# tranthai189765/MARL-Snake

Measured on AMD Instinct MI355X. Metric: env-steps/sec whole-node, 65536×(20×20, 4 snakes), random actions; 1→8 GPU, higher is better.
Workload: dtype u8

## Files before the change

marl-snake_amd/csrc/snake_capi.cpp:

```cpp
#include <stdarg.h>
#include <stdio.h>
#include <stdlib.h>
#include <string.h>

#include <math.h>

#include <algorithm>
#include <map>
#include <mutex>
#include <tuple>
#include <vector>

#include "snake_internal.h"

#ifndef SNAKE_SPAWN_PRIO_SMALL
#define SNAKE_SPAWN_PRIO_SMALL 3
#endif

namespace snake {

static thread_local char g_err[512];

void set_error(const char *fmt, ...)
{
    va_list ap;
    va_start(ap, fmt);
    vsnprintf(g_err, sizeof g_err, fmt, ap);
    va_end(ap);
}

static int64_t round_up(int64_t x, int64_t m) { return (x + m - 1) / m * m; }

static int pow2_at_least(int x)
{
    int p = 1;
    while (p < x) p <<= 1;
    return p;
}

static int check_cfg(const snake_cfg *c)
{
    if (!c) { set_error("cfg is NULL"); return SNAKE_E_CONFIG; }
    if (c->height < 3 || c->height > 255 || c->width < 3 || c->width > 255) {
        set_error("height/width must be in [3, 255] (got %d x %d)", c->height, c->width);
        return SNAKE_E_CONFIG;
    }
    if (c->num_snakes < 1 || c->num_snakes > kMaxSnakes) {
        set_error("num_snakes must be in [1, %d] (got %d)", kMaxSnakes, c->num_snakes);
        return SNAKE_E_CONFIG;
    }
    if (c->snake_length < 2 || c->snake_length > 63) {
        set_error("snake_length must be in [2, 63] (got %d)", c->snake_length);
        return SNAKE_E_CONFIG;
    }
    if (c->snake_length * c->num_snakes > kWave) {
        set_error("num_snakes * snake_length must be <= 64 (got %d)", c->snake_length * c->num_snakes);
        return SNAKE_E_CONFIG;
    }
    if (c->vision_range < 0 || 2 * c->vision_range + 1 > 255) {
        set_error("vision_range must be None/0 or in [1, 127] (got %d)", c->vision_range);
        return SNAKE_E_CONFIG;
    }
    if (c->frame_stack < 1 || c->frame_stack > 16) {
        set_error("frame_stack must be in [1, 16] (got %d)", c->frame_stack);
        return SNAKE_E_CONFIG;
    }
    if (c->observer != 0 && c->observer != 1) {
        set_error("observer must be 'snake' or 'human'");
        return SNAKE_E_CONFIG;
    }
    if (c->num_fruits < 1 || c->num_fruits > kMaxFruits) {
        set_error("num_fruits must be in [1, %d] (got %d)", kMaxFruits, c->num_fruits);
        return SNAKE_E_CONFIG;
    }
    int interior = (c->height - 2) * (c->width - 2);
    if (interior < c->num_snakes * c->snake_length + 1) {
        set_error("grid too small for %d snakes of length %d", c->num_snakes, c->snake_length);
        return SNAKE_E_CONFIG;
    }
    return SNAKE_OK;
}

struct Dfs {
    int H, W, L;
    std::vector<uint8_t> empty;
    std::vector<int16_t> *out;
    int64_t count = 0;
    int path[64];
    int dir_state[64];
};

static bool in_path(const Dfs &d, int n, int cell)
{
    for (int i = 0; i < n; i++)
        if (d.path[i] == cell) return true;
    return false;
}

static bool head_blocked(const Dfs &d, int n, int extra)
// ... 231 lines not shown
    }
    o->obs = N * S * oh * ow * 8 * fs;
    o->rew = N * S * 8;
    o->done = N * S;
    o->ep_done = N;
    o->rank = N * S * 4;
    o->ep_stats = N * 4 * S * 8;
    o->err = N * 4;
    if (o->n_cand > 65535) {
        set_error("%lld spawn poses: more than the 65535 the reset scratch indexes",
                  (long long)o->n_cand);
        return SNAKE_E_CONFIG;
    }
    if (o->n_cand < S) {
        set_error("only %lld spawn poses for %lld snakes", (long long)o->n_cand, (long long)S);
        return SNAKE_E_CONFIG;
    }
    int64_t samples = 0;
    const double pd = disjoint_prob(c->height, c->width, c->snake_length, (int)S, &samples);
    if (pd < kMinDisjoint) {
        set_error("%dx%d board too crowded: %lld snakes of length %d are disjoint in only "
                  "%.2g of the spawn draws (Monte-Carlo estimate: %lld of %lld sampled draws; the limit is %.0e; "
                  "the reference would retry ~%.0f permutations per reset)",
                  c->height, c->width, (long long)S, c->snake_length, pd, (long long)llround(pd * samples),
                  (long long)samples, kMinDisjoint, pd > 0 ? 1.0 / pd : 1e30);
        return SNAKE_E_CONFIG;
    }
    return SNAKE_OK;
}

int build_kcfg(const snake_cfg *c, int64_t N, int64_t n_cand, KCfg *k)
{
    snake_layout lay;
    int rc = layout_of(c, N, &lay);
    if (rc) return rc;
    if (n_cand != lay.n_cand) {
        set_error("spawn-pose table has %lld rows, expected %lld", (long long)n_cand,
                  (long long)lay.n_cand);
        return SNAKE_E_ARG;
    }
    memset(k, 0, sizeof *k);
    k->N = (int)N;
    k->H = c->height; k->W = c->width; k->HW = c->height * c->width;
    k->S = c->num_snakes; k->L = c->snake_length; k->vr = c->vision_range;
    k->fs = c->frame_stack; k->observer = c->observer; k->num_fruits = c->num_fruits;
    k->coop = c->coop ? 1 : 0; k->autoreset = c->autoreset == 2 ? 2 : (c->autoreset ? 1 : 0);
    k->oh = lay.obs_h; k->ow = lay.obs_w;
    k->units = k->S * k->oh * k->ow * k->fs;
    k->grid_stride = lay.grid_stride; k->ring_cap = lay.ring_cap; k->n_cand = (int)lay.n_cand;
    k->cs = (k->HW + kWave - 1) / kWave;
    k->ring_bytes = k->fs * k->grid_stride;
    int64_t a = 128;
    k->adv_f = (int)(a % k->fs); a /= k->fs;
    k->adv_j = (int)(a % k->ow); a /= k->ow;
    k->adv_i = (int)(a % k->oh); a /= k->oh;
    k->adv_k = (int)a;
    int off = 0;
    k->lds_frames = off; off += (int)round_up((int64_t)k->fs * k->grid_stride, 16);
    k->lds_centers = off; off += (int)round_up(4 * k->fs * kMaxSnakes, 16);
    k->lds_fruit = off; off += (int)round_up(2 * kMaxFruits, 16);
    {
        const int64_t P = (int64_t)k->oh * k->ow * 8 * k->fs;
        int g = 0;
        if ((int64_t)k->S * P <= kStageMax) {
            g = k->S;
        } else {
            g = (int)std::min<int64_t>(k->S, kStageMax / P);
            if (P % 16 != 0) g &= ~1;
        }
        k->enc_group = g;
        k->lds_stage = off;
        k->lds_worker = off;
        if (g > 0) off += (int)round_up(g * P, 16);
        const uint64_t fsoh = (uint64_t)k->fs * k->oh, oh = (uint64_t)k->oh;
        k->mag_fsoh = (uint32_t)(((1ull << 32) + fsoh - 1) / fsoh);
        k->mag_oh = (uint32_t)(((1ull << 32) + oh - 1) / oh);
        k->mag_W = (uint32_t)(((1ull << 32) + k->W - 1) / k->W);
        const uint64_t n16 = (uint64_t)k->grid_stride / 16;
        k->mag_n16 = (uint32_t)(((1ull << 32) + n16 - 1) / n16);
    }
    k->link_stride = (int)round_up(k->n_cand, 4) + kWave;
    int jbytes = (int)round_up(2 * ((int64_t)k->n_cand + kWave), 16);
    k->link_in_lds = jbytes <= kJarrLdsMax;
    if (k->link_in_lds && N <= 32768 && !bg_of(c, n_cand, N) && 4 * (int64_t)k->link_stride <= kJarrLdsMax) {
        k->link32 = 1;
        jbytes = 4 * k->link_stride;
    }
    k->reset_slots = (int)std::min<int64_t>(N, kResetSlots);
    const bool bg = bg_of(c, n_cand, N);
    const bool bg_small = bg && n_cand <= 8192 && N <= 8192;
    if (bg_small) k->reset_slots = (int)std::min<int64_t>(N, 512);
    k->spawn_prio = N <= 32768 && !bg ? SNAKE_SPAWN_PRIO_SMALL : 1;
    k->encode_prio = bg ? 0 : 2;
    {
        const int ms_min = k->S <= 4 ? 4 : (k->S <= 8 ? 8 : 16);
        k->logic_ms = N <= 8192 ? std::max(ms_min, 8) : ms_min;
    }
    auto logic_lds = [&](int G) {
        const int E = kWave / G;
        return (int)round_up((int64_t)E * k->grid_stride + 2 * kMaxFruits + E * G * 4 * 4 + E * G * 2, 16);
    };
    while (k->logic_ms < 16 && logic_lds(k->logic_ms) > kLdsLimit) k->logic_ms *= 2;
    k->lds_logic = logic_lds(k->logic_ms);
    if (k->lds_logic > kLdsLimit) {
        set_error("%dx%d board: k_logic's %d frames per wave (%d bytes) do not fit the %d-byte LDS", k->H, k->W,
                  kWave / k->logic_ms, k->lds_logic, kLdsLimit);
        return SNAKE_E_CONFIG;
    }
    k->logic_wpb = 4 * (int64_t)k->lds_logic <= kLdsLimit ? 4 : 1;
    k->q_envs_per_block = kWave / k->logic_ms;
    k->q_cap = (int)queue_cap(N, k->q_envs_per_block);
    k->spawn_thr = spawn_thr_of(c);
    if (bg_small && c->spawn_ahead == 0 && !c->coop && k->spawn_thr == 3) k->spawn_thr = 4;
    k->bg = bg ? 1 : 0;
    k->spawn_slots = (int)std::min<int64_t>(N, bg_small ? 512 : kResetSlots);
#ifndef SNAKE_BG_TRIES_SMALL
#define SNAKE_BG_TRIES_SMALL 2
#endif
    k->bg_tries = bg_small ? SNAKE_BG_TRIES_SMALL : 1;
    k->spawn_tries = 1;
    k->lds_obs_bytes = off;
    {
        const LeanGeom g = lean_geom(c);
        k->lean = g.lean; k->lp = g.lp; k->pw = g.pw; k->pframe = g.pframe;
        k->lds_lean_bytes = g.lds_lean_bytes; k->ups = g.ups; k->rowl = g.rowl;
        k->mag_ups = g.mag_ups; k->mag_rowl = g.mag_rowl; k->mag_fs = g.mag_fs; k->mag_wpr = g.mag_wpr;
        const int64_t fdw = (int64_t)k->fs * k->HW / 4;
        int t = 0;
        k->tbl_base = (int)round_up((int64_t)k->fs * k->pframe, 16); t = k->tbl_base + 8 * k->fs * kMaxSnakes;
        k->tbl_pat = t; t += 8 * k->S * 160;
        k->tbl_desc = t; t += (int)round_up(4 * (int64_t)k->units, 16);
        k->lds_tbl_bytes = t;
        k->tbl = g.exact && !g.lean && fdw <= 8 * kWave && t <= 40 * 1024 ? 1 : 0;
        if (g.lean && t <= 48 * 1024) k->tbl = 1;
    }
    k->enc_per_wave = k->lean ? 2 : (N >= 16384 && k->ring_bytes <= 8 * 1024 ? 2 : 1);
    if (k->tbl) k->enc_per_wave = k->lean ? 2 : 4;
    k->lds_link = k->lds_stage;
    k->lds_bytes = k->link_in_lds ? std::max(off, k->lds_stage + jbytes) : off;
    if (k->lds_bytes > 64 * 1024) {
        set_error("grid ring of %d bytes per env does not fit the LDS budget", k->ring_bytes);
        return SNAKE_E_CONFIG;
    }
    {
        const int E = kWave / k->logic_ms;
        k->nlg = (int)((N + E - 1) / E);
        k->fused = c->autoreset == 1 && k->tbl && !k->lean && !k->bg && k->fs == 1 && k->S <= 4 &&
                   k->enc_per_wave == 4 && E % 4 == 0 && (k->link32 || k->link_in_lds) ? 1 : 0;
        const int64_t fb = fused_base(N), groups = round_up((N + 3) / 4, 4);
        k->fu_ldone = fb;
        k->fu_done = fb + kQShards * kQSpread;
        k->fu_claim = k->fu_done + groups;
        k->fu_hoff = k->fu_claim + groups;
        k->epoch = 0;
    }
    k->rf = c->rew_fruit; k->rk = c->rew_kill; k->rl = c->rew_lose; k->rw = c->rew_win;
    k->rt = c->rew_time; k->max_steps = c->max_episode_steps;
    return SNAKE_OK;
}

static int check_state(const KCfg &k, const snake_state *st, bool need_all)
{
    if (!st || !st->grid || !st->snake || !st->body || !st->env || !st->ctr || !st->stats ||
        !st->mt || !st->cand) {
        set_error("snake_state has a NULL buffer");
        return SNAKE_E_ARG;
    }
    if (!st->resetq || !st->spawn) {
        set_error("snake_state.resetq / spawn is NULL");
        return SNAKE_E_ARG;
    }
    if ((!k.link_in_lds || (k.lean && k.autoreset == 1)) && !st->jscratch) {
        set_error("snake_state.jscratch is required for this config (n_cand=%d)", k.n_cand);
        return SNAKE_E_ARG;
    }
    (void)need_all;
    return SNAKE_OK;
}

static int check_out(const snake_out *o, bool step)
{
    if (!o || !o->obs) { set_error("snake_out.obs is NULL"); return SNAKE_E_ARG; }
    if (step && (!o->rew || !o->done || !o->ep_done || !o->rank || !o->ep_stats || !o->err)) {
        set_error("snake_out has a NULL step buffer");
        return SNAKE_E_ARG;
    }
    return SNAKE_OK;
}

static int64_t n_cand_of(const snake_cfg *c)
{
    snake_layout lay;
    if (layout_of(c, 1, &lay)) return -1;
    return lay.n_cand;
}

static int plan_cached(const snake_cfg *c, int64_t N, KCfg *k)
{
    struct Entry {
        snake_cfg cfg;
        int64_t n;
        KCfg k;
    };
    thread_local Entry memo[8];
    thread_local int used = 0, next = 0;
    if (!c) { set_error("cfg is NULL"); return SNAKE_E_CONFIG; }
    for (int i = 0; i < used; i++) {
        if (memo[i].n == N && memcmp(&memo[i].cfg, c, sizeof *c) == 0) {
            *k = memo[i].k;
            return SNAKE_OK;
        }
    }
    int rc = build_kcfg(c, N, n_cand_of(c), k);
    if (rc) return rc;
    Entry &e = memo[next];
    e.cfg = *c;
    e.n = N;
    e.k = *k;
    next = (next + 1) % 8;
    used = used < 8 ? used + 1 : 8;
    return SNAKE_OK;
}
// ... 103 lines not shown
```

marl-snake_amd/csrc/snake_internal.h:

```cpp
#pragma once
#include <stdint.h>

#include "../../include/snake_env.h"

namespace snake {

constexpr int kWave = 64;
constexpr int kMtN = 624;
constexpr int kMaxSnakes = 16;
constexpr int kMaxFruits = 64;
constexpr int kEnvRec = 8;
constexpr int kJarrLdsMax = 36864;
constexpr int kLdsLimit = 160 * 1024;
constexpr int kResetSlots = 2048;
constexpr int kQShards = 64;
constexpr int kStageMax = 8192;
constexpr int kSpawnStride = 672;
constexpr int kSpawnPos = 624;
constexpr int kSpawnCells = 625;
constexpr int kQSpread = 32;
constexpr int kClaimShards = 16;
constexpr int kNumQ = 3;
constexpr int kQClaim = kNumQ * kQShards;
constexpr int kQDone = kQClaim + kClaimShards;
constexpr int kQSpClaim = kQDone + 1;
constexpr int kQSpDone = kQSpClaim + kClaimShards;
constexpr int kQSpGen = kQSpDone + 1;
constexpr int kQCount = kQSpGen + 1;
constexpr int kQCounters = kQCount * kQSpread;
#ifndef SNAKE_QSETS
#define SNAKE_QSETS 4
#endif
constexpr int kQSets = SNAKE_QSETS;
static_assert(kQSets == 2 || kQSets == 4, "two or four queue sets");
constexpr int kQGenBits = 6;

enum { ENV_ALIVE = 0, ENV_EPLEN = 1, ENV_CUR = 2, ENV_MTPOS = 3, ENV_SPAWN = 4, ENV_FAIL = 5 };
constexpr int kSpawnBufShift = 2, kSpawnGenShift = 4;
enum { SPAWN_NONE = 0, SPAWN_PARTIAL = 1, SPAWN_READY = 2, SPAWN_DRAWING = 3 };

struct KCfg {
    int N;
    int H, W, HW, S, L, vr, fs, observer, num_fruits, coop, autoreset;
    int oh, ow, units;
    int grid_stride, ring_cap, n_cand;
    int cs;
    int ring_bytes;
    int adv_f, adv_j, adv_i, adv_k;
    int lds_frames, lds_centers, lds_fruit, lds_link, lds_bytes, link_in_lds;
    int link_stride;
    int link32;
    int lds_obs_bytes;
    int enc_group, lds_stage;
    uint32_t mag_fsoh, mag_oh;
    uint32_t mag_W;
    uint32_t mag_n16;
    int reset_slots;
    int logic_ms;
    int lds_logic;
    int logic_wpb;
    int q_envs_per_block;
    int q_cap;
    int spawn_thr;
    int spawn_prio;
    int encode_prio;
    int diag;
    int enc_per_wave;
    int bg;
    int lds_worker;
    int qpar;
    int spawn_slots;
    int bg_tries;
    int spawn_tries;
    uint32_t spawn_gate;
    int draw_wait;
    int spawn_delay;
    int lean, lp, pw, pframe, lds_lean_bytes, ups, rowl;
    int tbl, tbl_base, tbl_pat, tbl_desc, lds_tbl_bytes;
    uint32_t mag_ups, mag_rowl, mag_fs, mag_wpr;
    int fused, nlg, fu_roles;
    uint32_t epoch;
    int64_t fu_ldone, fu_done, fu_claim, fu_hoff;
    double rf, rk, rl, rw, rt, max_steps;
};

int build_kcfg(const snake_cfg *c, int64_t num_envs, int64_t n_cand, KCfg *k);
int layout_of(const snake_cfg *c, int64_t num_envs, snake_layout *out);
int64_t fused_base(int64_t num_envs);
int64_t fused_words(int64_t num_envs);
void set_error(const char *fmt, ...);

int launch_seed(const KCfg &k, const snake_state &st, uint32_t base_seed, int64_t env_offset,
                void *stream);
int launch_reset(const KCfg &k, const snake_state &st, const uint8_t *mask, const snake_out &o,
                 void *stream);
int launch_step(const KCfg &k, const snake_state &st, const int8_t *actions, const snake_out &o,
                void *stream);
int wait_background(const snake_state &st, void *stream);
int release_background(const snake_state &st);
int launch_render(const KCfg &k, const snake_state &st, const uint8_t *palette, uint8_t *rgb,
                  void *stream);

}
```

marl-snake_amd/csrc/snake_kernels.hip:

```cpp
#include <hip/hip_runtime.h>
#include <hip/hip_ext.h>

#include <limits.h>
#include <stdlib.h>
#include <string.h>

#include <map>
#include <string>
#include <vector>
#include <mutex>
#include <type_traits>
#include <utility>

#include "snake_internal.h"
#include "snake_device.h"
#include "snake_diag.h"

constexpr int kResetWavesPerEU = 4;

namespace snake {

enum { C_EMPTY = 0, C_WALL = 1, C_FRUIT = 2, C_HEAD = 3, C_BODY = 4, C_TAIL = 5 };

struct KArgs {
// ... 1789 lines not shown
        idx = G + x + nsh * nx;
    }
    const int jobs_x = T > G + x ? (T - G - x + nsh - 1) / nsh : 0;
    const int workers_x = (G - x + nsh - 1) / nsh;
    if (nx == jobs_x + workers_x - 1) {
        int d = 0;
        if (lane == 0) d = atomicAdd(&qc[kQSpDone * kQSpread], 1);
        if (bcast(d, 0) == nsh - 1) {
            for (int q = kQShards + lane; q < kNumQ * kQShards; q += kWave)
                st_sc1(reinterpret_cast<uint32_t *>(&qc[q * kQSpread]), 0u);
            if (lane <= kClaimShards) st_sc1(reinterpret_cast<uint32_t *>(&qc[(kQSpClaim + lane) * kQSpread]), 0u);
            __asm__ volatile("s_waitcnt vmcnt(0)" ::: "memory");
            if (lane == 0) atomicAdd(reinterpret_cast<unsigned *>(&qc[kQSpGen * kQSpread]), 1u);
        }
    }
}

__device__ __forceinline__ void encode_one(const KCfg &c, const snake_state &st, const snake_out &o, const int e)
{
    extern __shared__ __attribute__((aligned(16))) uint8_t lds[];
    const int lane = threadIdx.x;
    if (c.autoreset == 2 ? o.err[e] != 1 : (c.autoreset && o.ep_done[e])) return;
    if (c.encode_prio == 1) __builtin_amdgcn_s_setprio(1);
    else if (c.encode_prio == 2) __builtin_amdgcn_s_setprio(2);
    else if (c.encode_prio == 3) __builtin_amdgcn_s_setprio(3);
    encode_env(c, st, o, e, lds, lane);
}

__global__ void __launch_bounds__(64) k_encode(const KCfg c, const snake_state st, const snake_out o)
{
    encode_one(c, st, o, (int)blockIdx.x);
}

template <int NPF>
__device__ __forceinline__ void encode_multi(const KCfg &c, const snake_state &st, const snake_out &o, const int b)
{
    extern __shared__ __attribute__((aligned(16))) uint8_t lds[];
    const int lane = threadIdx.x;
    if (c.encode_prio == 1) __builtin_amdgcn_s_setprio(1);
    else if (c.encode_prio == 2) __builtin_amdgcn_s_setprio(2);
    else if (c.encode_prio == 3) __builtin_amdgcn_s_setprio(3);
    const int fs = c.fs, S = c.S, n16 = c.ring_bytes >> 4, fsS = fs * S;
    uint8_t *frames = lds + c.lds_frames;
    int *org = reinterpret_cast<int *>(lds + c.lds_centers);
    const int e_begin = b * c.enc_per_wave, e_end = min(c.N, e_begin + c.enc_per_wave);
    typedef uint32_t pf_t __attribute__((ext_vector_type(4 * NPF)));
    pf_t pf = {};
    int pcur = 0, pctr = 0, pskip = 0;
#define SNAKE_ENC_FETCH(EE)                                                                        \
    do {                                                                                           \
        const int64_t e_ = (EE);                                                                   \
        const uint4 *src_ = reinterpret_cast<const uint4 *>(st.grid + e_ * c.ring_bytes);          \
        _Pragma("unroll") for (int u = 0; u < NPF; u++) {      \
            const uint4 x_ = src_[min(lane + u * kWave, n16 - 1)];                                 \
            pf[4 * u] = x_.x; pf[4 * u + 1] = x_.y; pf[4 * u + 2] = x_.z; pf[4 * u + 3] = x_.w;     \
        }                                                                                          \
        pcur = st.env[e_ * kEnvRec + ENV_CUR];                                                     \
        pctr = lane < fsS ? st.ctr[e_ * fsS + lane] : 0;                                           \
        pskip = c.autoreset ? o.ep_done[e_] : 0;                                                   \
    } while (0)
    if (e_begin < e_end) SNAKE_ENC_FETCH(e_begin);
    for (int e = e_begin; e < e_end; e++) {
        const int cur = pcur, skip = pskip;
        if (!skip) {
            uint4 *d4 = reinterpret_cast<uint4 *>(frames);
#pragma unroll
            for (int u = 0; u < NPF; u++)
                d4[min(lane + u * kWave, n16 - 1)] = make_uint4(pf[4 * u], pf[4 * u + 1], pf[4 * u + 2], pf[4 * u + 3]);
            if (lane < fsS) {
                const int x = lane / S, k = lane - x * S;
                org[x * kMaxSnakes + k] = pack_origin(c, pctr >> 8, pctr & 255);
            }
        }
        if (e + 1 < e_end) SNAKE_ENC_FETCH(e + 1);
        if (!skip) {
            wave_sync();
            encode_obs(c, frames, org, cur + 1 == fs ? 0 : cur + 1, o.obs + (int64_t)e * c.units * 8, lds, lane);
            wave_sync();
        }
    }
#undef SNAKE_ENC_FETCH
}

constexpr int kPatV = 160;

template <int T>
__device__ __forceinline__ void tsync()
{
    if constexpr (T == kWave) wave_sync();
    else __syncthreads();
}

template <int NPW, int T = kWave, bool FU = false>
__device__ void encode_tbl_block(const KCfg &c, const snake_state &st, const snake_out &o, const int blk)
{
    extern __shared__ __attribute__((aligned(16))) uint8_t lds[];
    const int lane = threadIdx.x;
    if (c.encode_prio == 1) __builtin_amdgcn_s_setprio(1);
    else if (c.encode_prio == 2) __builtin_amdgcn_s_setprio(2);
    else if (c.encode_prio == 3) __builtin_amdgcn_s_setprio(3);
    uint8_t *pf = lds;
    uint2 *base = reinterpret_cast<uint2 *>(lds + c.tbl_base);
    uint8_t *pat = lds + c.tbl_pat;
    uint32_t *desc = reinterpret_cast<uint32_t *>(lds + c.tbl_desc);
    const int S = c.S, fs = c.fs, fsS = fs * S;
    const int wpr = c.W >> 2, nw = c.H * wpr, nwt = fs * nw, gsw = c.grid_stride >> 2;
    int src[NPW], dst[NPW];
#pragma unroll
    for (int u = 0; u < NPW; u++) {
        const int x = min(lane + u * T, nwt - 1);
        const int s = x / nw, xx = x - s * nw;
        const int r = fdiv((uint32_t)xx, c.mag_wpr, wpr), c4 = xx - r * wpr;
        src[u] = s * gsw + xx;
        dst[u] = (s * c.pframe + (r + c.vr) * c.pw + c.lp) / 4 + c4;
    }
    zero_lean<T>(c, pf, lane);
    const int npv = 3 + 3 * S;
    for (int x = lane; x < S * npv; x += T) {
        const int k = x / npv, r = x - k * npv;
        const int v = r < 3 ? r : 10 * ((r - 3) / 3) + 3 + (r - 3) % 3;
        const unsigned long long b = onehot(v, k);
        reinterpret_cast<uint2 *>(pat)[k * kPatV + v] = make_uint2((uint32_t)b, (uint32_t)(b >> 32));
    }
    for (int u = lane; u < c.units; u += T) {
        const int kk = (int)__umulhi((uint32_t)u, c.mag_ups), r0 = u - kk * c.ups;
        const int ii = (int)__umulhi((uint32_t)r0, c.mag_rowl), r1 = r0 - ii * c.rowl;
        const int jj = fdiv((uint32_t)r1, c.mag_fs, fs), ff = r1 - jj * fs;
        desc[u] = (uint32_t)(ii * c.pw + jj) | ((uint32_t)(ff * kMaxSnakes + kk) << 16);
    }
    const int e_begin = blk * c.enc_per_wave, e_end = min(c.N, e_begin + c.enc_per_wave);
    uint32_t w[NPW];
    int pcur = 0, pctr = 0, pskip = 0;
#define SNAKE_TBL_FETCH(EE)                                                                        \
    do {                                                                                           \
        const int64_t e_ = (EE);                                                                   \
        const uint32_t *r32_ = reinterpret_cast<const uint32_t *>(st.grid + e_ * c.ring_bytes);    \
        if constexpr (FU) {                                                                        \
            _Pragma("unroll") for (int u = 0; u < NPW; u++) w[u] = ld_sc1(r32_ + src[u]);          \
            const uint4 h_ = ld_sc1_128(st.resetq + c.fu_hoff + 4 * e_);                           \
            pcur = (int)(h_.x & 255u);                                                             \
            pskip = (int)((h_.x >> 8) & 1u);                                                       \
            pctr = lane < fsS ? (int)(((lane < 2 ? h_.y : h_.z) >> (16 * (lane & 1))) & 0xffffu) : 0; \
        } else {                                                                                   \
            _Pragma("unroll") for (int u = 0; u < NPW; u++) w[u] = r32_[src[u]];                   \
            pcur = st.env[e_ * kEnvRec + ENV_CUR];                                                 \
            pctr = lane < fsS ? st.ctr[e_ * fsS + lane] : 0;                                       \
            pskip = c.autoreset ? o.ep_done[e_] : 0;                                               \
        }                                                                                          \
    } while (0)
    if (e_begin < e_end) SNAKE_TBL_FETCH(e_begin);
    const int chunks = c.units >> 1;
    const bool one = T == kWave && chunks <= 4 * T;
    uint2 dr[4];
    if constexpr (T == kWave) if (one) {
        tsync<T>();
#pragma unroll
        for (int t = 0; t < 4; t++) dr[t] = reinterpret_cast<const uint2 *>(desc)[min(t * T + lane, chunks - 1)];
    }
    for (int e = e_begin; e < e_end; e++) {
        const int cur = pcur, skip = pskip;
        tsync<T>();
        if (!skip) {
#pragma unroll
            for (int u = 0; u < NPW; u++) reinterpret_cast<uint32_t *>(pf)[dst[u]] = w[u];
            if (lane < fsS) {
                const int s = lane / S, k = lane - s * S, slot0 = cur + 1 == fs ? 0 : cur + 1;
                const int f = s >= slot0 ? s - slot0 : s - slot0 + fs;
                const uint32_t gb = (uint32_t)(s * c.pframe) +
                                    (c.vr ? (uint32_t)((pctr >> 8) * c.pw + (pctr & 255) + c.lp - c.vr) : 0u);
                base[f * kMaxSnakes + k] = make_uint2(gb, (uint32_t)(k * kPatV * 8));
            }
        }
        if (e + 1 < e_end) SNAKE_TBL_FETCH(e + 1);
        if (!skip) {
            tsync<T>();
            const auto rs = __builtin_amdgcn_make_buffer_rsrc(o.obs + (int64_t)e * c.units * 8, 0, c.units * 8, 0x00020000);
            auto lookup = [&](uint2 dd) {
                const uint2 b0 = base[dd.x >> 16], b1 = base[dd.y >> 16];
                const uint32_t v0 = pf[b0.x + (dd.x & 0xffffu)], v1 = pf[b1.x + (dd.y & 0xffffu)];
                const uint2 p0 = *reinterpret_cast<const uint2 *>(pat + b0.y + 8 * v0);
                const uint2 p1 = *reinterpret_cast<const uint2 *>(pat + b1.y + 8 * v1);
                return (v4u){p0.x, p0.y, p1.x, p1.y};
            };
            if (T == kWave && one) {
                v4u r[4];
#pragma unroll
                for (int t = 0; t < 4; t++) r[t] = lookup(dr[t]);
#pragma unroll
                for (int t = 0; t < 4; t++)
                    if (t * T + lane < chunks) obs_store_rs(rs, 16 * (t * T + lane), r[t]);
            } else {
            constexpr int CP = T == kWave ? 4 : 2;
            for (int q0 = 0; q0 < chunks; q0 += CP * T) {
                v4u r[CP];
#pragma unroll
                for (int t = 0; t < CP; t++)
                    r[t] = lookup(reinterpret_cast<const uint2 *>(desc)[min(q0 + t * T + lane, chunks - 1)]);
#pragma unroll
                for (int t = 0; t < CP; t++)
                    if (q0 + t * T + lane < chunks) obs_store_rs(rs, 16 * (q0 + t * T + lane), r[t]);
            }
            }
        }
    }
#undef SNAKE_TBL_FETCH
}

constexpr unsigned long long kFuseWait = 10000000ull;
constexpr unsigned long long kFuseHelp = 2000ull;

__device__ __forceinline__ bool fused_claim(KPtr kp, const int g)
{
    const KCfg &c = kargs(kp).c;
    uint32_t *claim = reinterpret_cast<uint32_t *>(kargs(kp).st.resetq + c.fu_claim) + g;
    int won = 0;
    if ((threadIdx.x & (kWave - 1)) == 0) won = atomicExch(claim, c.epoch) != c.epoch ? 1 : 0;
    return __shfl(won, 0) != 0;
}

__device__ __forceinline__ bool fused_group_done(KPtr kp, const int g)
{
    const KCfg &c = kargs(kp).c;
    const uint32_t *done = reinterpret_cast<const uint32_t *>(kargs(kp).st.resetq + c.fu_done) + g;
    return (uint32_t)__shfl((int)ld_sc1(done), 0) == c.epoch;
}

__device__ __forceinline__ void fused_wait_group(KPtr kp, const int g)
{
    const unsigned long long t0 = __builtin_amdgcn_s_memrealtime();
    while (!fused_group_done(kp, g)) {
        if (__builtin_amdgcn_s_memrealtime() - t0 > kFuseWait) {
            if ((threadIdx.x & (kWave - 1)) == 0) DIAG_ADD(g_fused_timeout);
            return;
        }
        __builtin_amdgcn_s_sleep(4);
    }
}

__device__ __forceinline__ int fused_wait_all(KPtr kp, const int wid, const unsigned long long t0, int &scan)
{
    const int lane = threadIdx.x & (kWave - 1);
    for (;;) {
        const KCfg &c = kargs(kp).c;
        const int nlg = c.nlg;
        const uint32_t ns = lane < nlg ? (uint32_t)((nlg - lane + kQShards - 1) / kQShards) : 0u;
        const uint32_t v = ld_sc1(reinterpret_cast<const uint32_t *>(kargs(kp).st.resetq + c.fu_ldone) + lane * kQSpread);
        if (__ballot(v != c.epoch * ns) == 0ull) return -1;
        const unsigned long long dt = __builtin_amdgcn_s_memrealtime() - t0;
        if (dt > kFuseWait) {
            if (lane == 0) DIAG_ADD(g_fused_timeout);
            return -1;
        }
        if (dt > kFuseHelp && scan < nlg) {
            if (scan < 0) scan = 0;
            for (; scan < nlg; scan += kWave) {
                const int g = (wid * 61 + scan + lane) % nlg;
                const KCfg &c2 = kargs(kp).c;
                const uint32_t cl = scan + lane < nlg ? ld_sc1(reinterpret_cast<const uint32_t *>(kargs(kp).st.resetq + c2.fu_claim) + g)
                                                      : c2.epoch;
                unsigned long long m = __ballot(cl != c2.epoch);
                while (m) {
                    const int L = __ffsll((long long)m) - 1;
                    m &= m - 1;
                    const int gg = __shfl(g, L);
                    if (fused_claim(kp, gg)) return gg;
                }
            }
        }
        __builtin_amdgcn_s_sleep(8);
    }
}

template <int MS, int NPW, int JL>
__global__ void __launch_bounds__(64) __attribute__((amdgpu_waves_per_eu(4))) k_step(const KArgs)
{
    const KPtr kp = kernel_args();
    extern __shared__ __attribute__((aligned(16))) uint8_t lds[];
    PTIME(0);
    const int b = (int)blockIdx.x;
    const int nlg = kargs(kp).c.nlg, G = kargs(kp).c.reset_slots;
    const int roles = kargs(kp).c.fu_roles;
    const int role = b < nlg ? 0 : (b < nlg + G ? 1 : 2);
    if (!(roles & (1 << role))) return;
    const int j = b - nlg - G;
    const int eg = (4 * j) / (kWave / MS);
    const unsigned long long t0 = __builtin_amdgcn_s_memrealtime();
    int scan = -1;
    for (int it = 0;; it++) {
        int grp = -1;
        if (role == 0) {
            if (it == 0 && fused_claim(kp, b)) grp = b;
        } else if (role == 2) {
            if (it == 0 && !fused_group_done(kp, eg) && fused_claim(kp, eg)) grp = eg;
        } else {
            grp = fused_wait_all(kp, b - nlg, t0, scan);
        }
        if (grp < 0) break;
        LogicIn in;
        logic_load<MS, false>(kp, grp, in);
        logic_body<MS, false, true>(kp, grp, in);
        FDBG_MARK(3);
    }
    if (role == 0) { PTIME(1); return; }
    if (role == 1) {
        __builtin_amdgcn_fence(__ATOMIC_ACQUIRE, "agent");
        __asm__ volatile("s_waitcnt vmcnt(0)" ::: "memory");
        FDBG_MARK(4);
        autoreset_worker<4, false, JL>(kp, b - nlg, G, lds);
        FDBG_MARK(5);
        PTIME(1);
        return;
    }
    if (4 * j >= kargs(kp).c.N && FDBG_BAD(6, j)) return;
    fused_wait_group(kp, eg);
    FDBG_MARK(7);
    const KArgs &A = kargs(kp);
    encode_tbl_block<NPW, kWave, true>(A.c, A.st, A.o, j);
    PTIME(1);
}

template <int MS, int NPF, bool RO, int JL>
__global__ void __launch_bounds__(64) k_post(const KArgs)
{
    const KPtr kp = kernel_args();
    PTIME(0);
    const int G = kargs(kp).c.reset_slots, b = (int)blockIdx.x;
    if (b < G) {
        extern __shared__ __attribute__((aligned(16))) uint8_t lds[];
#ifdef SNAKE_DIAG_ENC2
        if (kargs(kp).aux) return;
#endif
        autoreset_worker<MS, RO, JL>(kp, b, G, lds);
    } else {
#ifdef SNAKE_DIAG_NO_ENCODE
        return;
#endif
        const KArgs &A = kargs(kp);
        if constexpr (NPF == 0) encode_one(A.c, A.st, A.o, b - G);
        else if constexpr (NPF < 0) encode_tbl_block<-NPF>(A.c, A.st, A.o, b - G);
        else encode_multi<NPF>(A.c, A.st, A.o, b - G);
    }
    PTIME(1);
}

template <int NPW, int T>
__device__ __forceinline__ void encode_lean_block(const KCfg &c, const snake_state &st, const snake_out &o,
                                                  const int blk)
{
    extern __shared__ __attribute__((aligned(16))) uint8_t lds[];
    const int lane = threadIdx.x;
    if (c.encode_prio == 1) __builtin_amdgcn_s_setprio(1);
    else if (c.encode_prio == 2) __builtin_amdgcn_s_setprio(2);
    else if (c.encode_prio == 3) __builtin_amdgcn_s_setprio(3);
    uint8_t *pf = lds;
    int *base = reinterpret_cast<int *>(lds + c.fs * c.pframe);
    uint32_t *p32 = reinterpret_cast<uint32_t *>(pf);
    const int wpr = c.W >> 2, nw = c.H * wpr, nwt = c.fs * nw, gsw = c.grid_stride >> 2, fsS = c.fs * c.S;
    auto sync = [&]() {
        if constexpr (T == kWave) wave_sync();
        else __syncthreads();
    };
    int src[NPW], dst[NPW];
#pragma unroll
    for (int u = 0; u < NPW; u++) {
        const int x = min(lane + u * T, nwt - 1);
        const int s = x / nw, xx = x - s * nw;
        const int r = fdiv((uint32_t)xx, c.mag_wpr, wpr), c4 = xx - r * wpr;
        src[u] = s * gsw + xx;
        dst[u] = (s * c.pframe + (r + c.vr) * c.pw + c.lp) / 4 + c4;
    }
    zero_lean<T>(c, pf, lane);
    const int e_begin = blk * c.enc_per_wave, e_end = min(c.N, e_begin + c.enc_per_wave);
    uint32_t w[NPW];
    int pcur = 0, pctr = 0, pskip = 0;
#define SNAKE_LEAN_FETCH(EE)                                                                       \
    do {                                                                                           \
        const int64_t e_ = (EE);                                                                   \
        const uint32_t *r32_ = reinterpret_cast<const uint32_t *>(st.grid + e_ * c.ring_bytes);    \
        _Pragma("unroll") for (int u = 0; u < NPW; u++) w[u] = r32_[src[u]];                       \
        pcur = st.env[e_ * kEnvRec + ENV_CUR];                                                     \
        pctr = lane < fsS ? st.ctr[e_ * fsS + lane] : 0;                                           \
        pskip = c.autoreset ? o.ep_done[e_] : 0;                                                   \
    } while (0)
    if (e_begin < e_end) SNAKE_LEAN_FETCH(e_begin);
    for (int e = e_begin; e < e_end; e++) {
        const int cur = pcur, skip = pskip;
        sync();
        if (!skip) {
#pragma unroll
            for (int u = 0; u < NPW; u++) p32[dst[u]] = w[u];
            if (lane < fsS) {
                const int x = lane / c.S, k = lane - x * c.S;
                base[x * kMaxSnakes + k] = c.vr ? (pctr >> 8) * c.pw + (pctr & 255) + c.lp - c.vr : 0;
            }
        }
        if (e + 1 < e_end) SNAKE_LEAN_FETCH(e + 1);
        if (!skip) {
            sync();
            encode_lean<T>(c, pf, base, cur + 1 == c.fs ? 0 : cur + 1, o.obs + (int64_t)e * c.units * 8, lane);
        }
    }
#undef SNAKE_LEAN_FETCH
}

template <int MS, bool RO, bool TBL>
__global__ void __launch_bounds__(256) k_post_lean(const KArgs)
{
    const KPtr kp = kernel_args();
    PTIME(0);
    extern __shared__ __attribute__((aligned(16))) uint8_t lds[];
    const int G = kargs(kp).c.reset_slots, GB = (G + 3) >> 2, b = (int)blockIdx.x;
    if (b < GB) {
        const int wave = (int)(threadIdx.x >> 6), wid = 4 * b + wave;
        if (wid < G) autoreset_worker<MS, RO, 0>(kp, wid, G, lds + wave * kargs(kp).c.lds_worker);
    } else {
        const KArgs &A = kargs(kp);
        if constexpr (TBL) encode_tbl_block<8, 256>(A.c, A.st, A.o, b - GB);
        else encode_lean_block<8, 256>(A.c, A.st, A.o, b - GB);
    }
    PTIME(1);
}

// ... 80 lines not shown
```

marl-snake_amd/csrc/snake_launch.inc:

```
namespace snake {

thread_local hipEvent_t t_ev0 = nullptr, t_ev1 = nullptr;
template <typename F, typename... Args>
static inline void slaunch(F kernel, const dim3 &grid, const dim3 &block, uint32_t lds, hipStream_t s,
                           Args... args)
{
    hipExtLaunchKernelGGL(kernel, grid, block, lds, s, t_ev0, t_ev1, 0u, args...);
}

namespace {
struct TimingRec {
    const char *name;
    hipEvent_t a, b;
};
std::mutex g_tmu;
bool g_timing = false;
int g_draw_wait_ticks = 200000;
int g_spawn_delay_ticks = 0;
int g_fuse_roles = 7;
#ifndef SNAKE_FUSED
#define SNAKE_FUSED 0
#endif
int g_fused = SNAKE_FUSED;
std::vector<TimingRec> g_pending;
// ... 118 lines not shown
{
    BgCtx c;
    {
        std::lock_guard<std::mutex> g(g_bgmu);
        g_fu.erase(st.env);
        auto it = g_bg.find(st.env);
        if (it == g_bg.end()) return SNAKE_OK;
        c = it->second;
        g_bg.erase(it);
    }
    DeviceGuard dg(c.x[0]);
    destroy_bg(c);
    return dg.dev < 0 ? SNAKE_E_LAUNCH : SNAKE_OK;
}

int launch_seed(const KCfg &k, const snake_state &st, uint32_t base_seed, int64_t env_offset, void *stream)
{
    const int threads = 256, blocks = (k.N + threads - 1) / threads;
    DeviceGuard dg((hipStream_t)stream);
    if (dg.dev < 0) return SNAKE_E_LAUNCH;
    if (int rc = wait_background(st, stream)) return rc;
    slaunch(k_seed, dim3(blocks), dim3(threads), 0, (hipStream_t)stream, k, st, base_seed, (long long)env_offset);
    return check_launch("k_seed");
}

int launch_render(const KCfg &k, const snake_state &st, const uint8_t *palette, uint8_t *rgb, void *stream)
{
    RenderPal pal;
    memcpy(pal.rgb, palette, sizeof(pal.rgb));
    DeviceGuard dg((hipStream_t)stream);
    if (dg.dev < 0) return SNAKE_E_LAUNCH;
    const long long quads = ((long long)k.N * k.HW + 3) / 4;
    const int threads = 256;
    const long long blocks = (quads + threads - 1) / threads;
    slaunch(k_render, dim3((unsigned)blocks), dim3(threads), 0, (hipStream_t)stream, k, st, pal, rgb);
    return check_launch("k_render");
}

template <int V> using Int = std::integral_constant<int, V>;
template <int... V, typename F>
static inline void pick(int v, F &&f)
{
    constexpr int list[] = {V...}, last = list[sizeof...(V) - 1];
    if (!((V != last && v == V ? (f(Int<V>{}), true) : false) || ...)) f(Int<last>{});
}
#define PICKED(x) decltype(x)::value

static inline int ms_of(int S) { return S <= 4 ? 4 : (S <= 8 ? 8 : 16); }
static inline int jl_of(const KCfg &k) { return k.link32 ? 2 : (k.link_in_lds ? 1 : 0); }

int launch_reset(const KCfg &k, const snake_state &st, const uint8_t *mask, const snake_out &o, void *stream)
{
    const dim3 grid(k.link_in_lds ? k.N : k.reset_slots), block(kWave);
    DeviceGuard dg((hipStream_t)stream);
    if (dg.dev < 0) return SNAKE_E_LAUNCH;
    if (int rc = wait_background(st, stream)) return rc;
    TimedLaunch tl("k_reset", (hipStream_t)stream);
    const KArgs a{k, st, o, mask};
    const hipStream_t s = (hipStream_t)stream;
    pick<0, 1, 2>(jl_of(k), [&](auto jl) {
        pick<4, 8, 16>(ms_of(k.S), [&](auto ms) {
            slaunch((k_reset<PICKED(ms), PICKED(jl)>), grid, block, k.lds_bytes, s, a);
        });
    });
    tl.close();
    return check_launch("k_reset");
}

struct PostShape {
    int npf;
    dim3 grid, block;
    int lds;
};

static PostShape post_shape(const KCfg &k)
{
    const int epw = k.enc_per_wave;
    if (k.lean)
        return {0, dim3((k.reset_slots + 3) / 4 + (k.N + epw - 1) / epw), dim3(256),
                std::max(4 * k.lds_worker, k.tbl ? k.lds_tbl_bytes : k.lds_lean_bytes)};
    const int n16 = k.ring_bytes >> 4;
    const int npw = (k.fs * k.HW / 4 + kWave - 1) / kWave;
    const int npf = k.tbl ? (npw <= 2 ? -2 : -8) : (epw <= 1 ? 0 : (n16 <= kWave ? 1 : (n16 <= 2 * kWave ? 2 : 8)));
    const int enc_blocks = npf == 0 ? k.N : (k.N + epw - 1) / epw;
    return {npf, dim3(k.reset_slots + enc_blocks), dim3(kWave),
            std::max(k.lds_bytes, k.tbl ? k.lds_tbl_bytes : k.lds_obs_bytes)};
}

static void launch_post(const KArgs &a, const PostShape &p, bool ro, int jl, hipStream_t s)
{
    if (a.c.lean)
        return pick<0, 1>(a.c.tbl ? 1 : 0, [&](auto tbl) {
            pick<0, 1>(a.c.bg ? 1 : 0, [&](auto bg) {
                pick<4, 8, 16>(ms_of(a.c.S), [&](auto ms) {
                    slaunch((k_post_lean<PICKED(ms), PICKED(bg) != 0, PICKED(tbl) != 0>), p.grid, p.block, p.lds, s, a);
                });
            });
        });
    auto go = [&](auto ro_c, auto jl_c) {
        pick<4, 8, 16>(ms_of(a.c.S), [&](auto ms) {
            pick<0, 1, 2, -2, -8, 8>(p.npf, [&](auto npf) {
                slaunch((k_post<PICKED(ms), PICKED(npf), PICKED(ro_c) != 0, PICKED(jl_c)>), p.grid, p.block, p.lds, s, a);
            });
        });
    };
    if (ro) go(Int<1>{}, Int<1>{});
    else pick<0, 1, 2>(jl, [&](auto jl_c) { go(Int<0>{}, jl_c); });
}

static int launch_encode(const KCfg &k, const snake_state &st, const snake_out &o, hipStream_t sm)
{
    TimedLaunch t3("k_encode", sm);
    slaunch(k_encode, dim3(k.N), dim3(kWave), k.lds_obs_bytes, sm, k, st, o);
    t3.close();
    return check_launch("k_encode");
}

static int launch_fused(KCfg &k, const snake_state &st, const int8_t *actions, const snake_out &o, hipStream_t sm)
{
    uint32_t ep;
    bool fresh = false;
    {
        std::lock_guard<std::mutex> g(g_bgmu);
        auto it = g_fu.find(st.env);
        if (it == g_fu.end()) { it = g_fu.emplace(st.env, 0u).first; fresh = true; }
        ep = it->second;
    }
    if (fresh && hipMemsetAsync(st.resetq + k.fu_ldone, 0, sizeof(int) * fused_words(k.N), sm) != hipSuccess) {
        set_error("zeroing the fused step's flags failed");
        return SNAKE_E_LAUNCH;
    }
    k.epoch = ep + 1;
    const int npw = (k.fs * k.HW / 4 + kWave - 1) / kWave;
    const dim3 gf(k.nlg + k.reset_slots + (k.N + 3) / 4), bf(kWave);
    const int lds_f = std::max(k.lds_logic, std::max(k.lds_bytes, k.lds_tbl_bytes));
    const KArgs fa{k, st, o, actions};
    TimedLaunch tf("k_step", sm);
    pick<4, 8>(k.logic_ms, [&](auto ms) {
        pick<2, 8>(npw <= 2 ? 2 : 8, [&](auto npw_c) {
            pick<2, 1>(k.link32 ? 2 : 1, [&](auto jl) {
                slaunch((k_step<PICKED(ms), PICKED(npw_c), PICKED(jl)>), gf, bf, lds_f, sm, fa);
            });
        });
    });
    tf.close();
    if (int rc = check_launch("k_step")) return rc;
    std::lock_guard<std::mutex> g(g_bgmu);
    g_fu[st.env] = ep + 1;
    return SNAKE_OK;
}

static int launch_logic(const KCfg &k, const snake_state &st, const int8_t *actions, const snake_out &o,
                        BgCtx *bgc, hipEvent_t &fork_ev, hipStream_t sm)
{
    TimedLaunch t1("k_logic", sm);
    if (bgc) {
        if (!t_ev1) t_ev1 = bgc->fork;
        fork_ev = t_ev1;
    }
    const KArgs la{k, st, o, actions};
    const unsigned epw = kWave / k.logic_ms, groups = (k.N + epw - 1) / epw;
    pick<4, 1>(k.logic_wpb, [&](auto wpb) {
        constexpr int WPB = PICKED(wpb);
        const dim3 glb((groups + WPB - 1) / WPB), blb(kWave * WPB);
        pick<0, 1>(k.bg ? 1 : 0, [&](auto bg) {
            pick<4, 8, 16>(k.logic_ms, [&](auto ms) {
                slaunch((k_logic<PICKED(ms), WPB, PICKED(bg) != 0>), glb, blb, WPB * k.lds_logic, sm, la);
            });
        });
// ... 165 lines not shown
```

Baseline: 819.1 million.

## Pack multiple table-encode waves per block and shrink per-wave encoder LDS

The table-based observation encoder now runs up to four waves per block, each with its own LDS slice. The pattern table is sized to the snake count, and descriptors are computed in registers when they fit, so per-wave LDS drops and more waves can be resident. The 32-bit link array is extended to N up to 65536 for the non-lean table path. Divisions are replaced with magic-number multiplies, and the first grid fetch is issued before table setup so its latency overlaps. The risks are wasted reset-slot blocks, since extra waves return immediately, and higher register pressure from the noinline encode path.

```diff
diff --git a/marl-snake_amd/csrc/snake_capi.cpp b/marl-snake_amd/csrc/snake_capi.cpp
--- a/marl-snake_amd/csrc/snake_capi.cpp
+++ b/marl-snake_amd/csrc/snake_capi.cpp
@@ -15,6 +15,12 @@
 
 #ifndef SNAKE_SPAWN_PRIO_SMALL
 #define SNAKE_SPAWN_PRIO_SMALL 3
+#endif
+#ifndef SNAKE_LINK32_MAX_ENVS
+#define SNAKE_LINK32_MAX_ENVS 65536
+#endif
+#ifndef SNAKE_TBL_EPW
+#define SNAKE_TBL_EPW 4
 #endif
 
 namespace snake {
@@ -412,10 +418,6 @@
     k->link_stride = (int)round_up(k->n_cand, 4) + kWave;
     int jbytes = (int)round_up(2 * ((int64_t)k->n_cand + kWave), 16);
     k->link_in_lds = jbytes <= kJarrLdsMax;
-    if (k->link_in_lds && N <= 32768 && !bg_of(c, n_cand, N) && 4 * (int64_t)k->link_stride <= kJarrLdsMax) {
-        k->link32 = 1;
-        jbytes = 4 * k->link_stride;
-    }
     k->reset_slots = (int)std::min<int64_t>(N, kResetSlots);
     const bool bg = bg_of(c, n_cand, N);
     const bool bg_small = bg && n_cand <= 8192 && N <= 8192;
@@ -458,16 +460,35 @@
         const int64_t fdw = (int64_t)k->fs * k->HW / 4;
         int t = 0;
         k->tbl_base = (int)round_up((int64_t)k->fs * k->pframe, 16); t = k->tbl_base + 8 * k->fs * kMaxSnakes;
-        k->tbl_pat = t; t += 8 * k->S * 160;
-        k->tbl_desc = t; t += (int)round_up(4 * (int64_t)k->units, 16);
-        k->lds_tbl_bytes = t;
-        k->tbl = g.exact && !g.lean && fdw <= 8 * kWave && t <= 40 * 1024 ? 1 : 0;
-        if (g.lean && t <= 48 * 1024) k->tbl = 1;
+        k->tbl_patv = 10 * k->S;
+        k->tbl_pat = t; t += 8 * k->S * k->tbl_patv;
+        k->tbl_desc = t;
+        if (g.lean || k->units / 2 > 4 * kWave) t += (int)round_up(4 * (int64_t)k->units, 16);
+        k->lds_tbl_bytes = (int)round_up(t, 16);
+        auto mag = [](uint64_t d) { return (uint32_t)(((1ull << 32) + d - 1) / d); };
+        k->mag_nw = mag((uint64_t)std::max(1, k->HW / 4));
+        k->mag_npv = mag(3 + 3 * (uint64_t)k->S);
+        k->mag_S = mag((uint64_t)k->S);
+        const int64_t t_full = k->tbl_pat + 8 * k->S * 160 + round_up(4 * (int64_t)k->units, 16);
+        k->tbl = g.exact && !g.lean && fdw <= 8 * kWave && t_full <= 40 * 1024 ? 1 : 0;
+        if (g.lean && t_full <= 48 * 1024) k->tbl = 1;
     }
     k->enc_per_wave = k->lean ? 2 : (N >= 16384 && k->ring_bytes <= 8 * 1024 ? 2 : 1);
-    if (k->tbl) k->enc_per_wave = k->lean ? 2 : 4;
+    if (k->tbl) k->enc_per_wave = k->lean ? 2 : SNAKE_TBL_EPW;
     k->lds_link = k->lds_stage;
+    if (k->link_in_lds && !bg && 4 * (int64_t)k->link_stride <= kJarrLdsMax &&
+        (N <= 32768 || (N <= SNAKE_LINK32_MAX_ENVS && k->tbl && !k->lean))) {
+        k->link32 = 1;
+        jbytes = 4 * k->link_stride;
+    }
     k->lds_bytes = k->link_in_lds ? std::max(off, k->lds_stage + jbytes) : off;
+#ifndef SNAKE_ENC_WPB
+#define SNAKE_ENC_WPB kEncWpbMax
+#endif
+    k->enc_wpb = 1;
+    if (k->tbl && !k->lean)
+        for (int w = 2; w <= std::min((int)SNAKE_ENC_WPB, kEncWpbMax); w++)
+            if (w * k->lds_tbl_bytes <= std::max(k->lds_bytes, 10 * 1024)) k->enc_wpb = w;
     if (k->lds_bytes > 64 * 1024) {
         set_error("grid ring of %d bytes per env does not fit the LDS budget", k->ring_bytes);
         return SNAKE_E_CONFIG;
diff --git a/marl-snake_amd/csrc/snake_internal.h b/marl-snake_amd/csrc/snake_internal.h
--- a/marl-snake_amd/csrc/snake_internal.h
+++ b/marl-snake_amd/csrc/snake_internal.h
@@ -13,6 +13,7 @@
 constexpr int kJarrLdsMax = 36864;
 constexpr int kLdsLimit = 160 * 1024;
 constexpr int kResetSlots = 2048;
+constexpr int kEncWpbMax = 4;
 constexpr int kQShards = 64;
 constexpr int kStageMax = 8192;
 constexpr int kSpawnStride = 672;
@@ -76,8 +77,10 @@
     int draw_wait;
     int spawn_delay;
     int lean, lp, pw, pframe, lds_lean_bytes, ups, rowl;
-    int tbl, tbl_base, tbl_pat, tbl_desc, lds_tbl_bytes;
+    int tbl, tbl_base, tbl_pat, tbl_patv, tbl_desc, lds_tbl_bytes;
+    int enc_wpb;
     uint32_t mag_ups, mag_rowl, mag_fs, mag_wpr;
+    uint32_t mag_nw, mag_npv, mag_S;
     int fused, nlg, fu_roles;
     uint32_t epoch;
     int64_t fu_ldone, fu_done, fu_claim, fu_hoff;
diff --git a/marl-snake_amd/csrc/snake_kernels.hip b/marl-snake_amd/csrc/snake_kernels.hip
--- a/marl-snake_amd/csrc/snake_kernels.hip
+++ b/marl-snake_amd/csrc/snake_kernels.hip
@@ -1895,8 +1895,6 @@
 #undef SNAKE_ENC_FETCH
 }
 
-constexpr int kPatV = 160;
-
 template <int T>
 __device__ __forceinline__ void tsync()
 {
@@ -1904,11 +1902,13 @@
     else __syncthreads();
 }
 
-template <int NPW, int T = kWave, bool FU = false>
-__device__ void encode_tbl_block(const KCfg &c, const snake_state &st, const snake_out &o, const int blk)
-{
-    extern __shared__ __attribute__((aligned(16))) uint8_t lds[];
-    const int lane = threadIdx.x;
+template <int NPW, int T, bool FU>
+__device__ __forceinline__ void encode_tbl_body(const KCfg &c, const snake_state &st, const snake_out &o, const int blk,
+                                                const int wave)
+{
+    extern __shared__ __attribute__((aligned(16))) uint8_t lds0[];
+    uint8_t *lds = lds0 + wave * c.lds_tbl_bytes;
+    const int lane = threadIdx.x & (T - 1);
     if (c.encode_prio == 1) __builtin_amdgcn_s_setprio(1);
     else if (c.encode_prio == 2) __builtin_amdgcn_s_setprio(2);
     else if (c.encode_prio == 3) __builtin_amdgcn_s_setprio(3);
@@ -1922,29 +1922,15 @@
 #pragma unroll
     for (int u = 0; u < NPW; u++) {
         const int x = min(lane + u * T, nwt - 1);
-        const int s = x / nw, xx = x - s * nw;
+        const int s = fdiv((uint32_t)x, c.mag_nw, nw), xx = x - s * nw;
         const int r = fdiv((uint32_t)xx, c.mag_wpr, wpr), c4 = xx - r * wpr;
         src[u] = s * gsw + xx;
         dst[u] = (s * c.pframe + (r + c.vr) * c.pw + c.lp) / 4 + c4;
     }
-    zero_lean<T>(c, pf, lane);
-    const int npv = 3 + 3 * S;
-    for (int x = lane; x < S * npv; x += T) {
-        const int k = x / npv, r = x - k * npv;
-        const int v = r < 3 ? r : 10 * ((r - 3) / 3) + 3 + (r - 3) % 3;
-        const unsigned long long b = onehot(v, k);
-        reinterpret_cast<uint2 *>(pat)[k * kPatV + v] = make_uint2((uint32_t)b, (uint32_t)(b >> 32));
-    }
-    for (int u = lane; u < c.units; u += T) {
-        const int kk = (int)__umulhi((uint32_t)u, c.mag_ups), r0 = u - kk * c.ups;
-        const int ii = (int)__umulhi((uint32_t)r0, c.mag_rowl), r1 = r0 - ii * c.rowl;
-        const int jj = fdiv((uint32_t)r1, c.mag_fs, fs), ff = r1 - jj * fs;
-        desc[u] = (uint32_t)(ii * c.pw + jj) | ((uint32_t)(ff * kMaxSnakes + kk) << 16);
-    }
     const int e_begin = blk * c.enc_per_wave, e_end = min(c.N, e_begin + c.enc_per_wave);
     uint32_t w[NPW];
     int pcur = 0, pctr = 0, pskip = 0;
-#define SNAKE_TBL_FETCH(EE)                                                                        \
+#define SNAKE_TBL_FETCH(EE)                                                                  \
     do {                                                                                           \
         const int64_t e_ = (EE);                                                                   \
         const uint32_t *r32_ = reinterpret_cast<const uint32_t *>(st.grid + e_ * c.ring_bytes);    \
@@ -1962,14 +1948,32 @@
         }                                                                                          \
     } while (0)
     if (e_begin < e_end) SNAKE_TBL_FETCH(e_begin);
+    zero_lean<T>(c, pf, lane);
+    const int npv = 3 + 3 * S, patv = c.tbl_patv;
+    for (int x = lane; x < S * npv; x += T) {
+        const int k = (int)__umulhi((uint32_t)x, c.mag_npv), r = x - k * npv;
+        const int v = r < 3 ? r : 10 * ((r - 3) / 3) + 3 + (r - 3) % 3;
+        const unsigned long long b = onehot(v, k);
+        reinterpret_cast<uint2 *>(pat)[k * patv + v] = make_uint2((uint32_t)b, (uint32_t)(b >> 32));
+    }
+    auto desc_of = [&](const int u) {
+        const int kk = (int)__umulhi((uint32_t)u, c.mag_ups), r0 = u - kk * c.ups;
+        const int ii = (int)__umulhi((uint32_t)r0, c.mag_rowl), r1 = r0 - ii * c.rowl;
+        const int jj = fdiv((uint32_t)r1, c.mag_fs, fs), ff = r1 - jj * fs;
+        return (uint32_t)(ii * c.pw + jj) | ((uint32_t)(ff * kMaxSnakes + kk) << 16);
+    };
     const int chunks = c.units >> 1;
     const bool one = T == kWave && chunks <= 4 * T;
     uint2 dr[4];
     if constexpr (T == kWave) if (one) {
-        tsync<T>();
-#pragma unroll
-        for (int t = 0; t < 4; t++) dr[t] = reinterpret_cast<const uint2 *>(desc)[min(t * T + lane, chunks - 1)];
-    }
+#pragma unroll
+        for (int t = 0; t < 4; t++) {
+            const int q = min(t * T + lane, chunks - 1);
+            dr[t] = make_uint2(desc_of(2 * q), desc_of(2 * q + 1));
+        }
+    }
+    if (!one)
+        for (int u = lane; u < c.units; u += T) desc[u] = desc_of(u);
     for (int e = e_begin; e < e_end; e++) {
         const int cur = pcur, skip = pskip;
         tsync<T>();
@@ -1977,11 +1981,11 @@
 #pragma unroll
             for (int u = 0; u < NPW; u++) reinterpret_cast<uint32_t *>(pf)[dst[u]] = w[u];
             if (lane < fsS) {
-                const int s = lane / S, k = lane - s * S, slot0 = cur + 1 == fs ? 0 : cur + 1;
+                const int s = fdiv((uint32_t)lane, c.mag_S, S), k = lane - s * S, slot0 = cur + 1 == fs ? 0 : cur + 1;
                 const int f = s >= slot0 ? s - slot0 : s - slot0 + fs;
                 const uint32_t gb = (uint32_t)(s * c.pframe) +
                                     (c.vr ? (uint32_t)((pctr >> 8) * c.pw + (pctr & 255) + c.lp - c.vr) : 0u);
-                base[f * kMaxSnakes + k] = make_uint2(gb, (uint32_t)(k * kPatV * 8));
+                base[f * kMaxSnakes + k] = make_uint2(gb, (uint32_t)(k * patv * 8));
             }
         }
         if (e + 1 < e_end) SNAKE_TBL_FETCH(e + 1);
@@ -2017,6 +2021,21 @@
         }
     }
 #undef SNAKE_TBL_FETCH
+}
+
+template <bool FU>
+__device__ __noinline__ void encode_tbl_block8(const KCfg &c, const snake_state &st, const snake_out &o, const int blk,
+                                               const int wave)
+{
+    encode_tbl_body<8, kWave, FU>(c, st, o, blk, wave);
+}
+
+template <int NPW, int T = kWave, bool FU = false>
+__device__ __forceinline__ void encode_tbl_block(const KCfg &c, const snake_state &st, const snake_out &o, const int blk,
+                                                 const int wave = 0)
+{
+    if constexpr (NPW == 8 && T == kWave) encode_tbl_block8<FU>(c, st, o, blk, wave);
+    else encode_tbl_body<NPW, T, FU>(c, st, o, blk, wave);
 }
 
 constexpr unsigned long long kFuseWait = 10000000ull;
@@ -2133,12 +2152,15 @@
 }
 
 template <int MS, int NPF, bool RO, int JL>
-__global__ void __launch_bounds__(64) k_post(const KArgs)
+__global__ void __launch_bounds__(NPF < 0 ? kWave * kEncWpbMax : kWave) k_post(const KArgs)
 {
     const KPtr kp = kernel_args();
     PTIME(0);
     const int G = kargs(kp).c.reset_slots, b = (int)blockIdx.x;
+    int wave = 0;
+    if constexpr (NPF < 0) wave = __builtin_amdgcn_readfirstlane((int)(threadIdx.x >> 6));
     if (b < G) {
+        if (wave) return;
         extern __shared__ __attribute__((aligned(16))) uint8_t lds[];
 #ifdef SNAKE_DIAG_ENC2
         if (kargs(kp).aux) return;
@@ -2150,7 +2172,11 @@
 #endif
         const KArgs &A = kargs(kp);
         if constexpr (NPF == 0) encode_one(A.c, A.st, A.o, b - G);
-        else if constexpr (NPF < 0) encode_tbl_block<-NPF>(A.c, A.st, A.o, b - G);
+        else if constexpr (NPF < 0) {
+            const int grp = (b - G) * A.c.enc_wpb + wave;
+            if (grp * A.c.enc_per_wave >= A.c.N) return;
+            encode_tbl_block<-NPF>(A.c, A.st, A.o, grp, wave);
+        }
         else encode_multi<NPF>(A.c, A.st, A.o, b - G);
     }
     PTIME(1);
diff --git a/marl-snake_amd/csrc/snake_launch.inc b/marl-snake_amd/csrc/snake_launch.inc
--- a/marl-snake_amd/csrc/snake_launch.inc
+++ b/marl-snake_amd/csrc/snake_launch.inc
@@ -224,9 +224,10 @@
     const int n16 = k.ring_bytes >> 4;
     const int npw = (k.fs * k.HW / 4 + kWave - 1) / kWave;
     const int npf = k.tbl ? (npw <= 2 ? -2 : -8) : (epw <= 1 ? 0 : (n16 <= kWave ? 1 : (n16 <= 2 * kWave ? 2 : 8)));
-    const int enc_blocks = npf == 0 ? k.N : (k.N + epw - 1) / epw;
-    return {npf, dim3(k.reset_slots + enc_blocks), dim3(kWave),
-            std::max(k.lds_bytes, k.tbl ? k.lds_tbl_bytes : k.lds_obs_bytes)};
+    const int enc_waves = npf == 0 ? k.N : (k.N + epw - 1) / epw;
+    const int wpb = k.tbl ? k.enc_wpb : 1;
+    return {npf, dim3(k.reset_slots + (enc_waves + wpb - 1) / wpb), dim3(kWave * wpb),
+            std::max(k.lds_bytes, k.tbl ? wpb * k.lds_tbl_bytes : k.lds_obs_bytes)};
 }
 
 static void launch_post(const KArgs &a, const PostShape &p, bool ro, int jl, hipStream_t s)
```

Measured after the change: 846.2 million, median of 6. +3.3%, better.
